# adammoss/nnest

Hardware: AMD Instinct MI355X
Metric: live-point evals/sec (flow-transform + loglike) + log-Z error, x_dim=50 (higher is better)
Workload: dtype f32

## Files before the change

### nnest_amd/csrc/nnest_train_grid.h

```cpp

enum { GRID_WG = 8, GRID_MAX_POLLS = 1 << 22 };

__device__ __forceinline__ void st_sc1_f32x4(float *p, f32x4 v) {
    asm volatile("global_store_dwordx4 %0, %1, off sc1\n\ts_nop 1" : : "v"(p), "v"(v) : "memory");
}
__device__ __forceinline__ float ld_sc1(const float *p) { return __hip_atomic_load(p, __ATOMIC_RELAXED, __HIP_MEMORY_SCOPE_AGENT); }
__device__ __forceinline__ f32x4 ld_sc1_x4_issue(const float *p) {
    f32x4 v;
    asm volatile("global_load_dwordx4 %0, %1, off sc1" : "=v"(v) : "v"(p) : "memory");
    return v;
}
__device__ __forceinline__ void st_sc1(float *p, float v) { __hip_atomic_store(p, v, __ATOMIC_RELAXED, __HIP_MEMORY_SCOPE_AGENT); }

__device__ __forceinline__ bool grid_barrier(unsigned int *ctr, int &phase, int G, int *err, int first_poll_sleep = 0) {
    asm volatile("s_waitcnt vmcnt(0)" ::: "memory");
    __syncthreads();
    phase += 1;
    __shared__ int ok;
    if (threadIdx.x == 0) {
        __hip_atomic_fetch_add(ctr, 1u, __ATOMIC_RELAXED, __HIP_MEMORY_SCOPE_AGENT);
        const unsigned int want = (unsigned int)G * (unsigned int)phase;
        int polls = 0, good = 1;
        if (first_poll_sleep >= 256) {
            for (int i = 256; i < first_poll_sleep; ++i) __builtin_amdgcn_s_sleep(4);
        } else if (first_poll_sleep > 8) __builtin_amdgcn_s_sleep(16);
        else if (first_poll_sleep > 0) __builtin_amdgcn_s_sleep(8);
        while (__hip_atomic_load(ctr, __ATOMIC_RELAXED, __HIP_MEMORY_SCOPE_AGENT) < want) {
            if (++polls > GRID_MAX_POLLS) { good = 0; *err = 1; break; }
            __builtin_amdgcn_s_sleep(1);
        }
        ok = good;
    }
    __syncthreads();
    return ok != 0;
}

template <int NT, int NH, int L>
__host__ __device__ inline void grid_job_targets(const FlowShape &s, int J, int lane, int r, int *wt, int *bt) {
    constexpr int J_W3 = NT * NH, J_W2 = L * NH * NH, NJOBS = J_W3 + J_W2 + NH * NT;
    const int D = s.D, H = s.H;
    const int bn = J / NJOBS, b = bn >> 1;
    int q = J % NJOBS;
    const int pc = (b + 1) & 1, pt = b & 1;
    const int pb0 = H * D, phid = H * D + H, pWo = H * D + H + L * (H * H + H), pbo = pWo + D * H;
    const int pbase = bn * s.net_params;
    const int gq = lane >> 4, j = lane & 15;
    *wt = -1; *bt = -1;
    if (q < J_W3) {
        const int tau = q / NH, ht = q % NH, d = 2 * (16 * tau + 4 * gq + r) + pt;
        if (d < D) {
            *wt = pbase + pWo + d * H + 16 * ht + j;
            if (ht == 0 && j == 0) *bt = pbase + pbo + d;
        }
        return;
    }
    q -= J_W3;
    if (q < J_W2) {
        const int l = q / (NH * NH) + 1, hto = (q / NH) % NH, hti = q % NH;
        *wt = pbase + phid + (l - 1) * (H * H + H) + (16 * hto + 4 * gq + r) * H + 16 * hti + j;
        if (hti == 0 && j == 0) *bt = pbase + phid + (l - 1) * (H * H + H) + H * H + 16 * hto + 4 * gq + r;
        return;
    }
    q -= J_W2;
    const int ht = q / NT, tau = q % NT, d = 2 * (16 * tau + j) + pc;
    if (d < D) *wt = pbase + (16 * ht + 4 * gq + r) * D + d;
    if (tau == 0 && j == 0) *bt = pbase + pb0 + 16 * ht + 4 * gq + r;
}

template <int NT, int NH, int L>
__global__ void grid_gpos_kernel(int *__restrict__ gpos, FlowShape s) {
    constexpr int NJOBS = NT * NH + L * NH * NH + NH * NT;
    const int NJ = s.B * 2 * NJOBS;
    for (int i = blockIdx.x * blockDim.x + threadIdx.x; i < NJ * 256; i += gridDim.x * blockDim.x) {
        const int J = i >> 8, lane = (i >> 2) & 63, r = i & 3;
        int wt, bt;
        grid_job_targets<NT, NH, L>(s, J, lane, r, &wt, &bt);
        if (wt >= 0) gpos[wt] = i;
        if (bt >= 0) gpos[bt] = NJ * 256 + i;
    }
}

template <int NT, int NH, int L>
__host__ __device__ inline void grid_job_image_offsets(const FlowShape &s, int J, int *off_f, int *off_b, int *off_bias) {
    constexpr int J_W3 = NT * NH, J_W2 = L * NH * NH, NJOBS = J_W3 + J_W2 + NH * NT;
    const int bn = J / NJOBS, base = bn * s.net_floats;
    int q = J % NJOBS;
    if (q < J_W3) {
        const int tau = q / NH, ht = q % NH;
        *off_b = base + frag_off_L1() + (ht * NT + tau) * 256;
        *off_f = base + frag_off_L3(NT, NH, L) + (tau * NH + ht) * 256;
        *off_bias = ht == 0 ? base + frag_off_b3(NT, NH, L) + 16 * tau : -1;
        return;
    }
    q -= J_W3;
    if (q < J_W2) {
        const int l = q / (NH * NH), hto = (q / NH) % NH, hti = q % NH;
        *off_b = base + frag_off_L2(NT, NH) + ((l * NH + hti) * NH + hto) * 256;
        *off_f = base + frag_off_L2(NT, NH) + ((l * NH + hto) * NH + hti) * 256;
        *off_bias = hti == 0 ? base + frag_off_b2(NT, NH, L) + l * 16 * NH + 16 * hto : -1;
        return;
    }
    q -= J_W2;
    const int ht = q / NT, tau = q % NT;
    *off_b = base + frag_off_L3(NT, NH, L) + (tau * NH + ht) * 256;
    *off_f = base + frag_off_L1() + (ht * NT + tau) * 256;
    *off_bias = tau == 0 ? base + frag_off_b1(NT, NH, L) + 16 * ht : -1;
}
__global__ void grid_dead_kernel(const int *__restrict__ gpos, int np, int *__restrict__ dead, int *__restrict__ count) {
    for (int p = blockIdx.x * blockDim.x + threadIdx.x; p < np; p += gridDim.x * blockDim.x)
        if (gpos[p] < 0) dead[atomicAdd(count, 1)] = p;
}

template <bool WITH_BIAS>
__device__ __forceinline__ f32x4 contract_rows_grid(const float *stg, int rows_pad, int ct_g, int ct_a, int lane, f32x4 &bias) {
    const f32x4 zero4 = {0.f, 0.f, 0.f, 0.f};
    f32x4 a0 = zero4, a1 = zero4, a2 = zero4, a3 = zero4;
    float bs = 0.f;
    const float *G = stg + (size_t)ct_g * TRAIN_MAX_ROWS * 16 + (lane >> 4) * 16 + (lane & 15);
    const float *A = stg + (size_t)ct_a * TRAIN_MAX_ROWS * 16 + (lane >> 4) * 16 + (lane & 15);
    constexpr int NIT = TRAIN_MAX_ROWS / 16;
    float gv[NIT][4], ev[NIT][4];
#pragma unroll
    for (int it = 0; it < NIT; ++it) {
        const int r = it * 16 < rows_pad ? it * 16 : 0;
#pragma unroll
        for (int k = 0; k < 4; ++k) {
            gv[it][k] = ld_sc1(G + (r + 4 * k) * 16);
            ev[it][k] = ld_sc1(A + (r + 4 * k) * 16);
        }
    }
#pragma unroll
    for (int it = 0; it < NIT; ++it) {
        if (it * 16 < rows_pad) {
            a0 = mfma4(gv[it][0], ev[it][0], a0);
            a1 = mfma4(gv[it][1], ev[it][1], a1);
            a2 = mfma4(gv[it][2], ev[it][2], a2);
            a3 = mfma4(gv[it][3], ev[it][3], a3);
            if (WITH_BIAS) bs += (gv[it][0] + gv[it][1]) + (gv[it][2] + gv[it][3]);
        }
    }
    if (WITH_BIAS) {
        bs += __shfl_xor(bs, 16);
        bs += __shfl_xor(bs, 32);
        const int q4 = (lane >> 4) * 4;
        bias = (f32x4){__shfl(bs, q4 + 0), __shfl(bs, q4 + 1), __shfl(bs, q4 + 2), __shfl(bs, q4 + 3)};
    }
    return (a0 + a1) + (a2 + a3);
}

__device__ __forceinline__ void stage_tile_grid(float *stg, int ct, int row, int lane, f32x4 v) {
    st_sc1_f32x4(stg + ((size_t)ct * TRAIN_MAX_ROWS + row) * 16 + (lane >> 4) * 4, v);
}

template <int NT, int NH, int L, int ACT>
__device__ __forceinline__ void mlp_bwd_grid(const float *__restrict__ bn, int lane, float *stg, int row, const f32x4 (&g_out)[NT],
                                             const f32x4 (&acts)[L + 1][NH], f32x4 (&g_m)[NT]) {
    typedef StageMap<NT, NH, L> SM;
    const float *B3 = bn + frag_off_L1() + 4 * lane;
    const float *B2 = bn + frag_off_L2(NT, NH) + 4 * lane;
    const float *B1 = bn + frag_off_L3(NT, NH, L) + 4 * lane;
    f32x4 gh[NH];
#pragma unroll
    for (int tau = 0; tau < NT; ++tau) stage_tile_grid(stg, SM::gout(tau), row, lane, g_out[tau]);
#pragma unroll
    for (int ht = 0; ht < NH; ++ht) {
        f32x4 acc = {0.f, 0.f, 0.f, 0.f};
#pragma unroll
        for (int tau = 0; tau < NT; ++tau) {
            const f32x4 f = frag_quad(B3, (ht * NT + tau));
            acc = mfma4(f.x, g_out[tau].x, acc);
            acc = mfma4(f.y, g_out[tau].y, acc);
            acc = mfma4(f.z, g_out[tau].z, acc);
            acc = mfma4(f.w, g_out[tau].w, acc);
        }
        gh[ht] = acc;
    }
#pragma unroll
    for (int l = L; l >= 1; --l) {
        f32x4 gpre[NH];
#pragma unroll
        for (int ht = 0; ht < NH; ++ht) {
            gpre[ht] = act_grad<ACT>(gh[ht], acts[l][ht]);
            stage_tile_grid(stg, SM::gpre(l, ht), row, lane, gpre[ht]);
            stage_tile_grid(stg, SM::act(l, ht), row, lane, acts[l][ht]);
        }
#pragma unroll
        for (int hti = 0; hti < NH; ++hti) {
            f32x4 acc = {0.f, 0.f, 0.f, 0.f};
#pragma unroll
            for (int hto = 0; hto < NH; ++hto) {
                const f32x4 f = frag_quad(B2, (((l - 1) * NH + hti) * NH + hto));
                acc = mfma4(f.x, gpre[hto].x, acc);
                acc = mfma4(f.y, gpre[hto].y, acc);
                acc = mfma4(f.z, gpre[hto].z, acc);
                acc = mfma4(f.w, gpre[hto].w, acc);
            }
            gh[hti] = acc;
        }
    }
    f32x4 gpre0[NH];
#pragma unroll
    for (int ht = 0; ht < NH; ++ht) {
        gpre0[ht] = act_grad<ACT>(gh[ht], acts[0][ht]);
        stage_tile_grid(stg, SM::gpre(0, ht), row, lane, gpre0[ht]);
        stage_tile_grid(stg, SM::act(0, ht), row, lane, acts[0][ht]);
    }
#pragma unroll
    for (int tau = 0; tau < NT; ++tau) {
        f32x4 acc = {0.f, 0.f, 0.f, 0.f};
#pragma unroll
        for (int ht = 0; ht < NH; ++ht) {
            const f32x4 f = frag_quad(B1, (tau * NH + ht));
            acc = mfma4(f.x, gpre0[ht].x, acc);
            acc = mfma4(f.y, gpre0[ht].y, acc);
            acc = mfma4(f.z, gpre0[ht].z, acc);
            acc = mfma4(f.w, gpre0[ht].w, acc);
        }
        g_m[tau] = acc;
    }
}

template <int NT, int NH, int L>
__device__ __forceinline__ void block_backward_grid(const TrainArgs &a, int b, int lane, int row, bool row_ok, const f32x4 (&cond)[NT],
                                                    f32x4 (&ytrans)[NT], f32x4 (&gcond)[NT], f32x4 (&gtrans)[NT], float gld,
                                                    const float *imgf, const float *imgb, const f32x4 *__restrict__ stash) {
    typedef StageMap<NT, NH, L> SM;
    const int pt = b & 1;
    const float *wf = imgf + (size_t)b * 2 * a.s.net_floats;
    const float *wb = imgb + (size_t)b * 2 * a.s.net_floats;
    float *stg_s = a.gstage + (size_t)(b * 2 + 0) * SM::count * TRAIN_MAX_ROWS * 16;
    float *stg_t = a.gstage + (size_t)(b * 2 + 1) * SM::count * TRAIN_MAX_ROWS * 16;
    f32x4 as[L + 1][NH], at[L + 1][NH], ls[NT], t[NT], g_ls[NT], g_t[NT], gm_s[NT], gm_t[NT];
    const int g = lane >> 4;
#pragma unroll
    for (int l = 0; l <= L; ++l)
#pragma unroll
        for (int ht = 0; ht < NH; ++ht) {
            as[l][ht] = stash[((0 * (L + 1) + l) * NH + ht) * 64 + lane];
            at[l][ht] = stash[((1 * (L + 1) + l) * NH + ht) * 64 + lane];
        }
    mlp_out_layer<NT, NH, L>(wf, lane, as[L], ls);
    mlp_out_layer<NT, NH, L>(wf + a.s.net_floats, lane, at[L], t);
#pragma unroll
    for (int tau = 0; tau < NT; ++tau) {
        float lsv[4] = {ls[tau].x, ls[tau].y, ls[tau].z, ls[tau].w};
        float tv[4] = {t[tau].x, t[tau].y, t[tau].z, t[tau].w};
        float yv[4] = {ytrans[tau].x, ytrans[tau].y, ytrans[tau].z, ytrans[tau].w};
        float gv[4] = {gtrans[tau].x, gtrans[tau].y, gtrans[tau].z, gtrans[tau].w};
        float o_gls[4], o_gt[4], o_x[4], o_gx[4];
#pragma unroll
        for (int r = 0; r < 4; ++r) {
            const int d = 2 * (16 * tau + 4 * g + r) + pt;
            const bool valid = row_ok && d < a.s.D;
            float ymt = yv[r] - tv[r];
            o_gls[r] = valid ? gv[r] * ymt + gld : 0.f;
            o_gt[r] = valid ? gv[r] : 0.f;
            o_x[r] = ymt * __expf(-lsv[r]);
            o_gx[r] = gv[r] * __expf(lsv[r]);
        }
        g_ls[tau] = (f32x4){o_gls[0], o_gls[1], o_gls[2], o_gls[3]};
        g_t[tau] = (f32x4){o_gt[0], o_gt[1], o_gt[2], o_gt[3]};
        ytrans[tau] = (f32x4){o_x[0], o_x[1], o_x[2], o_x[3]};
        gtrans[tau] = (f32x4){o_gx[0], o_gx[1], o_gx[2], o_gx[3]};
    }
    mlp_bwd_grid<NT, NH, L, 0>(wb, lane, stg_s, row, g_ls, as, gm_s);
#pragma unroll
    for (int tau = 0; tau < NT; ++tau) {
        f32x4 mv = cond[tau];
        if (!row_ok) mv = (f32x4){0.f, 0.f, 0.f, 0.f};
        stage_tile_grid(stg_s, SM::m(tau), row, lane, mv);
        stage_tile_grid(stg_t, SM::m(tau), row, lane, mv);
    }
    mlp_bwd_grid<NT, NH, L, 1>(wb + a.s.net_floats, lane, stg_t, row, g_t, at, gm_t);
#pragma unroll
    for (int tau = 0; tau < NT; ++tau) gcond[tau] = gcond[tau] + gm_s[tau] + gm_t[tau];
}

__device__ __forceinline__ void lds_barrier_t() { asm volatile("s_waitcnt lgkmcnt(0)\n\ts_barrier" ::: "memory"); }

template <int NT>
__device__ __forceinline__ void team_swap(f32x4 *xch, int role, int lane, const f32x4 (&mine)[NT], f32x4 (&other)[NT]) {
#pragma unroll
    for (int tau = 0; tau < NT; ++tau) xch[(role * NT + tau) * 64 + lane] = mine[tau];
// ... 571 lines not shown
```

### nnest_amd/csrc/nnest_train_rows.h

```cpp

enum { ROWS_PER_WG = 4, ROWS_B = 3 };

template <int U> struct RowsKeep {
    float h1, h2;
    float ls[(U + 1) / 2], tt[(U + 1) / 2];
};

__device__ __forceinline__ int rows_img_off(int b, int f, int lane) { return b * SOLO4_NF * 64 + ((f >> 2) * 64 + lane) * 4 + (f & 3); }

template <int U>
__device__ inline void rows_param_dest(int D, int b, int n, int o, int &df, int &db, bool &scaled) {
    const int cc = (b + 1) & 1, ct = b & 1;
    const int pb0 = 16 * D, pW1 = pb0 + 16, pb1 = pW1 + 256, pWo = pb1 + 16, pbo = pWo + 16 * D;
    df = db = -1;
    scaled = false;
    auto lane_of = [&](int pos, int src) { const int dl = (pos - src) & 15; return 32 * n + 16 * (dl >> 3) + pos; };
    auto rot_of = [&](int pos, int src) { return ((pos - src) & 15) & 7; };
    if (o < pb0) {
        const int j = o / D, d = o % D;
        if ((d & 1) != cc) return;
        const int s = d >> 1, q = s / U, u = s % U;
        df = rows_img_off(b, 8 * u + rot_of(j, q), lane_of(j, q));
        db = rows_img_off(b, 40 + 8 * u + rot_of(q, j), lane_of(q, j));
        scaled = n == 0;
// ... 100 lines not shown

static __device__ __forceinline__ float rows_act_grad(float g, float a, unsigned sel) {
    const float th = g * (1.f - a * a), rl = a > 0.f ? g : 0.f;
    unsigned out;
    asm("v_bfi_b32 %0, %1, %2, %3" : "=v"(out) : "v"(sel), "v"(__float_as_uint(rl)), "v"(__float_as_uint(th)));
    return __uint_as_float(out);
}

static __device__ __forceinline__ void rows_stage(float *stg_net, int ct, int row, int col, float v, bool stager) {
    if (stager) st_sc1(stg_net + ((size_t)ct * TRAIN_MAX_ROWS + row) * 16 + col, v);
}
template <int U>
static __device__ __forceinline__ void rows_stage_slots(float *stg_net, int ct0, int row, int pos, const float (&v)[U], bool stager) {
    if constexpr (U == 4) {
        const int s = 4 * pos;
        if (stager) st_sc1_f32x4(stg_net + ((size_t)(ct0 + (s >> 4)) * TRAIN_MAX_ROWS + row) * 16 + (s & 15), (f32x4){v[0], v[1], v[2], v[3]});
    } else {
#pragma unroll
        for (int u = 0; u < U; ++u) {
            const int s = U * pos + u;
            rows_stage(stg_net, ct0 + (s >> 4), row, s & 15, v[u], stager);
        }
    }
}

template <int U>
static __device__ __forceinline__ void rows_block_backward(const Solo4Lds &wb_, unsigned sel, bool h1, bool translate_half, int pos, int D, int ct,
                                                           bool row_ok, float gld, const float (&cond)[U], float (&ytrans)[U], float (&gcond)[U],
                                                           float (&gtrans)[U], const RowsKeep<U> &kp, float *stg_net, int row, bool stager) {
    typedef StageMap<U, 1, 1> SM;
    float go[U];
#pragma unroll
    for (int k = 0; k < U / 2; ++k) {
        const int u = 2 * k + (h1 ? 1 : 0);
        const bool valid = row_ok && 2 * U * pos + 2 * u + ct < D;
        const float yv = h1 ? ytrans[2 * k + 1] : ytrans[2 * k], gv = h1 ? gtrans[2 * k + 1] : gtrans[2 * k];
        const float ymt = yv - kp.tt[k];
        const float g_ls = valid ? gv * ymt + gld : 0.f, g_t = valid ? gv : 0.f;
        float x0 = ymt * __expf(-kp.ls[k]), gx0 = gv * __expf(kp.ls[k]), gs0 = translate_half ? g_t : g_ls;
        float x1 = x0, gx1 = gx0, gs1 = gs0;
        solo_swap16(x0, x1);
        solo_swap16(gx0, gx1);
        solo_swap16(gs0, gs1);
        ytrans[2 * k] = x0; ytrans[2 * k + 1] = x1;
        gtrans[2 * k] = gx0; gtrans[2 * k + 1] = gx1;
        go[2 * k] = gs0; go[2 * k + 1] = gs1;
    }
    if constexpr (U & 1) {
        const bool valid = row_ok && 2 * U * pos + 2 * (U - 1) + ct < D;
        const float gv = gtrans[U - 1], ymt = ytrans[U - 1] - kp.tt[U / 2];
        const float g_ls = valid ? gv * ymt + gld : 0.f, g_t = valid ? gv : 0.f;
        ytrans[U - 1] = ymt * __expf(-kp.ls[U / 2]);
        gtrans[U - 1] = gv * __expf(kp.ls[U / 2]);
        go[U - 1] = translate_half ? g_t : g_ls;
    }
    rows_stage_slots<U>(stg_net, SM::gout(0), row, pos, go, stager);
    float wa[8], wb[8], a0, a1;
    if constexpr (U >= 2) {
        wb_.load8(wa, 0); wb_.load8(wb, 8);
        solo_chain_2in(a0, a1, 0.f, solo_rot8_h1(go[0]), solo_rot8_h1(go[U >= 2 ? 1 : 0]), wa, wb);
    }
    if constexpr (U == 4) {
        wb_.load8(wa, 16); wb_.load8(wb, 24);
        solo_chain_2in_acc(a0, a1, solo_rot8_h1(go[U == 4 ? 2 : 0]), solo_rot8_h1(go[U == 4 ? 3 : 0]), wa, wb);
    }
    if constexpr (U == 1) {
        wb_.load8(wa, 0);
        solo_chain_1(a0, a1, 0.f, solo_rot8_h1(go[0]), wa);
    }
    if constexpr (U == 3) {
        wb_.load8(wa, 16);
        solo_chain_1_acc(a0, a1, solo_rot8_h1(go[U - 1]), wa);
    }
    float w2[8], w3a[8], w3b[8];
    wb_.load8(w2, 32);
    const float g_a2 = rows_act_grad(solo_join_rot(a0 + a1), kp.h2, sel);
    rows_stage(stg_net, SM::gpre(1, 0), row, pos, g_a2, stager);
    rows_stage(stg_net, SM::act(1, 0), row, pos, kp.h2, stager);
    if constexpr (U >= 2) { wb_.load8(w3a, 40); wb_.load8(w3b, 48); }
    solo_chain_1(a0, a1, 0.f, g_a2, w2);
    const float g_a1 = rows_act_grad(solo_join_rot(a0 + a1), kp.h1, sel);
    rows_stage(stg_net, SM::gpre(0, 0), row, pos, g_a1, stager);
    rows_stage(stg_net, SM::act(0, 0), row, pos, kp.h1, stager);
    {
        float cm[U];
#pragma unroll
        for (int u = 0; u < U; ++u) cm[u] = row_ok ? cond[u] : 0.f;
        rows_stage_slots<U>(stg_net, SM::m(0), row, pos, cm, stager);
    }
#pragma unroll
    for (int k = 0; k < U / 2; ++k) {
        float o0, o1;
        if (k > 0) { wb_.load8(w3a, 40 + 16 * k); wb_.load8(w3b, 48 + 16 * k); }
        solo_chain_2out(o0, o1, 0.f, 0.f, g_a1, w3a, w3b);
        solo_swap16(o0, o1);
        float fs, ft;
        solo_nets(o0 + o1, fs, ft);
        float t0 = fs + ft, t1 = t0;
        solo_swap16(t0, t1);
        gcond[2 * k] += t0;
        gcond[2 * k + 1] += t1;
    }
    if constexpr (U & 1) {
        float o0, o1;
        wb_.load8(wa, 40 + 8 * (U - 1));
        solo_chain_1(o0, o1, 0.f, g_a1, wa);
        float fs, ft;
        solo_nets(solo_join(o0 + o1), fs, ft);
        gcond[U - 1] += fs + ft;
    }
}

template <int U>
__device__ __forceinline__ void rows_prepare(const TrainArgs &a, int epoch, int mb, int wg, float *buf) {
    const int idx = (int)threadIdx.x - 64 * ROWS_PER_WG;
    if (idx < 0 || idx >= ROWS_PER_WG * 8 * U) return;
    const int r = idx / (8 * U), q = idx % (8 * U), D = a.s.D;
    const int M = min(a.batch, a.n_train - mb * a.batch);
    const int row = wg * ROWS_PER_WG + r;
    const bool row_ok = row < M;
    long src = 0;
    if (row_ok) src = a.perm[(size_t)epoch * a.n_train + mb * a.batch + row];
    const int d0 = 4 * q;
    float v[4];
#pragma unroll
    for (int j = 0; j < 4; ++j) v[j] = (row_ok && d0 + j < D) ? a.xtrain[(size_t)src * D + d0 + j] : 0.f;
    if (a.jitter != 0.f && row_ok) {
        const long p = (long)mb * a.batch + row;
        float n[4];
        if (a.noise) {
#pragma unroll
            for (int j = 0; j < 4; ++j) n[j] = d0 + j < D ? a.noise[((size_t)epoch * a.n_train + p) * D + d0 + j] : 0.f;
        } else {
            const f32x4 nn = noise_normal4(a.seed, (uint64_t)p, (uint32_t)(a.epoch_offset + epoch), (uint32_t)q, NOISE_STREAM_JITTER);
            n[0] = nn.x; n[1] = nn.y; n[2] = nn.z; n[3] = nn.w;
        }
#pragma unroll
        for (int j = 0; j < 4; ++j)
            if (d0 + j < D) v[j] += n[j] * a.jitter;
    }
    *reinterpret_cast<f32x4 *>(buf + r * 32 * U + d0) = (f32x4){v[0], v[1], v[2], v[3]};
}

template <int U>
__global__ void __launch_bounds__(TRAIN_THREADS) train_kernel_rows(TrainArgs a) {
    typedef StageMap<U, 1, 1> SM;
    constexpr int B = ROWS_B, IMG = ROWS_B * SOLO4_NF * 64;
    extern __shared__ __attribute__((aligned(16))) float smem[];
    float *imgf = smem;
    float *imgb = smem + IMG;
    __shared__ __attribute__((aligned(16))) float xpre[2][ROWS_PER_WG * 32 * U];
    __shared__ int ctl[4];
    __shared__ float ctlf[2];
    const int lane = threadIdx.x & 63, wave = threadIdx.x >> 6;
    const int pos = lane & 15;
    const bool h1 = (lane & 16) != 0, translate_half = lane >= 32, stager = (lane & 16) == 0;
    const int sl_r = (int)a.gld_in & 255, sl_b = ((int)a.gld_in >> 8) & 255;
    const unsigned sel = translate_half ? 0xffffffffu : 0u;
    const int wg = blockIdx.x, G = gridDim.x;
    const int D = a.s.D;
    constexpr int NJOBS = 2 * U + 1;
    const int NJ = B * 2 * NJOBS;
    int phase = 0;

    for (int i = threadIdx.x; i < 2 * IMG; i += blockDim.x) smem[i] = 0.f;
    __syncthreads();
    for (int p = threadIdx.x; p < a.s.nets_params(); p += blockDim.x) {
        const int bn = p / a.s.net_params, o = p - bn * a.s.net_params;
        int df, db; bool sc;
        rows_param_dest<U>(D, bn >> 1, bn & 1, o, df, db, sc);
        const float v = a.w[p];
        if (df >= 0) imgf[df] = sc ? SOLO_TANH_PRESCALE * v : v;
        if (db >= 0) imgb[db] = v;
    }
    constexpr int IMGF = ROWS_B * 2 * (2 * U * 256 + 256 + 16 + 16 + 16 * U);
    constexpr int RU = (IMGF / 4 + TRAIN_THREADS - 1) / TRAIN_THREADS;
    typedef int i32x4 __attribute__((ext_vector_type(4)));
    const i32x4 *gmap = reinterpret_cast<const i32x4 *>(a.gown);
    static_assert(2 * IMG < 0xffff && IMG < (1 << 14), "refresh map packing");

    const int Jmine = wave * G + wg;
    const bool owner = Jmine < NJ;
    int off_f = 0, off_b = 0, off_bias = -1;
    if (owner) grid_job_image_offsets<U, 1, 1>(a.s, Jmine, &off_f, &off_b, &off_bias);
    OwnState os;
#pragma unroll
    for (int r = 0; r < 4; ++r) {
        os.wt[r] = os.bt[r] = -1;
        os.tw[r] = os.tm[r] = os.tv[r] = os.bw[r] = os.bm[r] = os.bv[r] = 0.f;
    }
    if (owner) {
#pragma unroll
        for (int r = 0; r < 4; ++r) {
            grid_job_targets<U, 1, 1>(a.s, Jmine, lane, r, &os.wt[r], &os.bt[r]);
            if (os.wt[r] >= 0) { os.tw[r] = a.w[os.wt[r]]; os.tm[r] = a.m[os.wt[r]]; os.tv[r] = a.v[os.wt[r]]; }
            if (os.bt[r] >= 0) { os.bw[r] = a.w[os.bt[r]]; os.bm[r] = a.m[os.bt[r]]; os.bv[r] = a.v[os.bt[r]]; }
        }
    }
    const int n_waves = G * TRAIN_WAVES, ndead = *a.gndead;
    const int ndead_pad = (ndead + 63) & ~63;
    const int dead_per = ((ndead + n_waves - 1) / n_waves + 63) & ~63;
    const int dead0 = min(ndead, Jmine * dead_per), dead1 = min(ndead, dead0 + dead_per);
    float *dw = a.gdst, *dm = a.gdst + ndead_pad, *dv = a.gdst + 2 * ndead_pad;
    for (int k = dead0 + lane; k < dead1; k += 64) {
        const int pidx = a.gdead[k];
        dw[k] = a.w[pidx]; dm[k] = a.m[pidx]; dv[k] = a.v[pidx];
    }
    const bool resume = (a.flags & NNEST_TRAIN_RESUME) != 0;
    if (threadIdx.x == 0) {
        ctl[0] = 0;
        ctl[1] = resume ? a.result->counter : 0;
        ctl[2] = resume ? a.result->best_epoch : 0;
        ctlf[0] = resume ? a.result->best_validation_loss : INFINITY;
    }
    if (!resume) {
        if (owner) {
#pragma unroll
            for (int r = 0; r < 4; ++r) {
                if (os.wt[r] >= 0) st_sc1(a.best_w + os.wt[r], os.tw[r]);
                if (os.bt[r] >= 0) st_sc1(a.best_w + os.bt[r], os.bw[r]);
            }
        }
        for (int k = dead0 + lane; k < dead1; k += 64) st_sc1(a.best_w + a.gdead[k], dw[k]);
    }
    const int n_mb = (a.n_train + a.batch - 1) / a.batch;
    if (a.max_epochs > 0) rows_prepare<U>(a, 0, 0, wg, xpre[0]);
    __syncthreads();

    float *pub = a.gimgf;
    float *part_base = a.gtile;
    auto sum_rows = [&](const float *words) {
        float v = (lane < ROWS_PER_WG * G ? ld_sc1(words + lane) : 0.f) + (lane + 64 < ROWS_PER_WG * G ? ld_sc1(words + lane + 64) : 0.f);
#pragma unroll
        for (int o = 1; o < 64; o <<= 1) v += __shfl_xor(v, o);
        return v;
    };
    int adam_t = a.adam_step ? *a.adam_step : 0;
    unsigned long long ph[8] = {0, 0, 0, 0, 0, 0, 0, 0}, q0 = 0, q1 = 0, q2 = 0, q3 = 0, q4 = 0, q5 = 0, q6 = 0;
    (void)ph; (void)q0; (void)q1; (void)q2; (void)q3; (void)q4; (void)q5; (void)q6;
    int epochs_run = 0, mbcount = 0;
    float last_train_loss = 0.f;
    bool alive = true;
    unsigned long long dbg_arr = 0, dbg_st = 0;
    (void)dbg_arr; (void)dbg_st;
    const int row = wg * ROWS_PER_WG + wave;
    float *stg_net0 = a.gstage + (size_t)(translate_half ? 1 : 0) * SM::count * TRAIN_MAX_ROWS * 16;

    auto forward = [&](float (&xs)[2][U], RowsKeep<U> (&kp)[B]) {
        float ld = rows_block_forward<U>(Solo4Lds{imgf, lane}, sel, h1, xs[1], xs[0], kp[0]);
        ld += rows_block_forward<U>(Solo4Lds{imgf + SOLO4_NF * 64, lane}, sel, h1, xs[0], xs[1], kp[1]);
        ld += rows_block_forward<U>(Solo4Lds{imgf + 2 * SOLO4_NF * 64, lane}, sel, h1, xs[1], xs[0], kp[2]);
        return ld;
    };
    auto log_prob = [&](const float (&xs)[2][U], float ld_lane) {
        float ss = 0.f;
#pragma unroll
        for (int c = 0; c < 2; ++c)
#pragma unroll
            for (int u = 0; u < U; ++u) ss += base_E(xs[c][u], a.s.base_beta);
        return -solo_row_sum(ss) + a.s.base_const * (float)D + solo_logdet_total(ld_lane);
    };

    for (int epoch = 0; epoch < a.max_epochs && alive; ++epoch) {
        float epoch_loss = 0.f;
        for (int mb = 0; mb < n_mb && alive; ++mb, ++mbcount) {
            const int M = min(a.batch, a.n_train - mb * a.batch);
            const int rows_pad = ((M + 15) >> 4) * 16;
            const bool row_ok = wave < ROWS_PER_WG && row < M;
            float *part = part_base + (mbcount & 1) * TRAIN_MAX_ROWS;
            AdamStep ad;
            {
                adam_t += 1;
                const double bc1 = 1.0 - pow(0.9, (double)adam_t), bc2 = 1.0 - pow(0.999, (double)adam_t);
                ad.step_size = (float)((double)a.lr / bc1);
                ad.inv_bc2s = (float)(1.0 / sqrt(bc2));
            }
            TSTAMP(q0);
#ifdef NNEST_STAMP
            const unsigned long long rt_start = __builtin_amdgcn_s_memrealtime();
#endif
            {
                int e2 = epoch, m2 = mb + 1;
                if (m2 == n_mb) { m2 = 0; e2 = epoch + 1; }
                if (e2 < a.max_epochs) rows_prepare<U>(a, e2, m2, wg, xpre[(mbcount + 1) & 1]);
            }
            if (wave < ROWS_PER_WG) {
                float lp = 0.f;
                if (row < rows_pad) {
                    float xs[2][U], gs[2][U];
                    const float *xr = xpre[mbcount & 1] + wave * 32 * U + 2 * U * pos;
#pragma unroll
                    for (int u = 0; u < U; ++u) { xs[0][u] = xr[2 * u]; xs[1][u] = xr[2 * u + 1]; }
                    RowsKeep<U> kp[B];
                    const float ld_lane = forward(xs, kp);
                    lp = row_ok ? log_prob(xs, ld_lane) : 0.f;
                    TSTAMP(q1);
                    const float invM = 1.0f / (float)M, gld = -invM;
#pragma unroll
                    for (int c = 0; c < 2; ++c)
#pragma unroll
                        for (int u = 0; u < U; ++u) gs[c][u] = row_ok ? base_dE(xs[c][u], a.s.base_beta) * invM : 0.f;
                    constexpr size_t RS = (size_t)2 * SM::count * TRAIN_MAX_ROWS * 16;
                    rows_block_backward<U>(Solo4Lds{imgb + 2 * SOLO4_NF * 64, lane}, sel, h1, translate_half, pos, D, 0, row_ok, gld, xs[1], xs[0], gs[1], gs[0], kp[2], stg_net0 + 2 * RS, row, stager);
                    rows_block_backward<U>(Solo4Lds{imgb + SOLO4_NF * 64, lane}, sel, h1, translate_half, pos, D, 1, row_ok, gld, xs[0], xs[1], gs[0], gs[1], kp[1], stg_net0 + RS, row, stager);
                    rows_block_backward<U>(Solo4Lds{imgb, lane}, sel, h1, translate_half, pos, D, 0, row_ok, gld, xs[1], xs[0], gs[1], gs[0], kp[0], stg_net0, row, stager);
                }
                if (lane == 0) st_sc1(part + row, lp);
            }
            TSTAMP(q2);
#ifdef NNEST_STAMP
            if (mbcount == 20) { dbg_arr = __builtin_amdgcn_s_memrealtime(); dbg_st = rt_start; }
#endif
#ifdef NNEST_STAMP
            {
                unsigned long long s0 = 0, s1 = 0;
                TSTAMP(s0);
                asm volatile("s_waitcnt vmcnt(0)" ::: "memory");
                __syncthreads();
                TSTAMP(s1);
                phase += 1;
                __shared__ int okd;
                if (threadIdx.x == 0) {
                    __hip_atomic_fetch_add(a.gsync, 1u, __ATOMIC_RELAXED, __HIP_MEMORY_SCOPE_AGENT);
                    const unsigned int want = (unsigned int)G * (unsigned int)phase;
                    int polls = 0;
                    __builtin_amdgcn_s_sleep(16);
                    while (__hip_atomic_load(a.gsync, __ATOMIC_RELAXED, __HIP_MEMORY_SCOPE_AGENT) < want) { ++polls; __builtin_amdgcn_s_sleep(1); }
                    okd = 1;
                    TACC(ph[6], s1, s0);
                    ph[7] += polls;
                }
                __syncthreads();
                alive = okd != 0;
            }
#else
            alive = grid_barrier(a.gsync, phase, G, a.gerr, 256 + sl_b);
#endif
            if (!alive) break;
            TSTAMP(q3);
            if (owner) {
                const int J = Jmine;
                const int bn = J / NJOBS;
                int q = J % NJOBS;
                const float *stg = a.gstage + (size_t)bn * SM::count * TRAIN_MAX_ROWS * 16;
                f32x4 bt = {0.f, 0.f, 0.f, 0.f}, t;
                constexpr int J_W3 = U, J_W2 = 1;
                if (q < J_W3) {
                    t = contract_rows_grid<true>(stg, rows_pad, SM::gout(q), SM::act(1, 0), lane, bt);
                } else if (q - J_W3 < J_W2) {
                    t = contract_rows_grid<true>(stg, rows_pad, SM::gpre(1, 0), SM::act(0, 0), lane, bt);
                } else {
                    q -= J_W3 + J_W2;
                    t = q == 0 ? contract_rows_grid<true>(stg, rows_pad, SM::gpre(0, 0), SM::m(q), lane, bt)
                               : contract_rows_grid<false>(stg, rows_pad, SM::gpre(0, 0), SM::m(q), lane, bt);
                }
                const float gt[4] = {t.x, t.y, t.z, t.w}, gb[4] = {bt.x, bt.y, bt.z, bt.w};
#pragma unroll
                for (int r = 0; r < 4; ++r) {
                    if (os.wt[r] >= 0) adam_reg(a, ad, os.tw[r], gt[r], os.tm[r], os.tv[r]);
                    if (os.bt[r] >= 0) adam_reg(a, ad, os.bw[r], gb[r], os.bm[r], os.bv[r]);
                }
                const float tg = __int_as_float(mbcount + 1);
                st_sc1_f32x4(pub + 2 * (off_b + lane * 4), (f32x4){os.tw[0], tg, os.tw[1], tg});
                st_sc1_f32x4(pub + 2 * (off_b + lane * 4) + 4, (f32x4){os.tw[2], tg, os.tw[3], tg});
                if (off_bias >= 0 && (lane & 15) == 0) {
                    st_sc1_f32x4(pub + 2 * (off_bias + (lane >> 4) * 4), (f32x4){os.bw[0], tg, os.bw[1], tg});
                    st_sc1_f32x4(pub + 2 * (off_bias + (lane >> 4) * 4) + 4, (f32x4){os.bw[2], tg, os.bw[3], tg});
                }
            }
            for (int k = dead0 + lane; k < dead1; k += 64) {
                float w_ = dw[k], m_ = dm[k], v_ = dv[k];
                adam_reg(a, ad, w_, 0.f, m_, v_);
                dw[k] = w_; dm[k] = m_; dv[k] = v_;
            }
            TSTAMP(q4);
            __syncthreads();
            TSTAMP(q5);
            float lsum = 0.f;
            if (wave == 0) lsum = sum_rows(part);
            {
                constexpr int CH = RU > 4 ? 4 : RU;
                const int want = mbcount + 1;
                for (int i = 0; i < sl_r; ++i) __builtin_amdgcn_s_sleep(4);
#pragma unroll
                for (int c0 = 0; c0 < RU; c0 += CH) {
                    f32x4 va[CH], vc[CH];
                    i32x4 mp[CH];
#pragma unroll
                    for (int u = 0; u < CH; ++u) mp[u] = gmap[min((int)threadIdx.x + (c0 + u) * TRAIN_THREADS, IMGF / 4 - 1)];
                    bool fresh = false;
                    for (int polls = 0; !fresh; ++polls) {
                        if (polls > GRID_MAX_POLLS / 64) { *a.gerr = 1; break; }
#pragma unroll
                        for (int u = 0; u < CH; ++u) {
                            const int i = min((int)threadIdx.x + (c0 + u) * TRAIN_THREADS, IMGF / 4 - 1);
                            va[u] = ld_sc1_x4_issue(pub + 8 * (size_t)i);
                            vc[u] = ld_sc1_x4_issue(pub + 8 * (size_t)i + 4);
                        }
#pragma unroll
                        for (int u = 0; u < CH; ++u) asm volatile("s_waitcnt vmcnt(0)" : "+v"(va[u]), "+v"(vc[u]) : : "memory");
                        fresh = true;
#pragma unroll
                        for (int u = 0; u < CH; ++u)
                            fresh = fresh && __float_as_int(va[u].y) == want && __float_as_int(va[u].w) == want && __float_as_int(vc[u].y) == want &&
                                    __float_as_int(vc[u].w) == want;
                    }
#pragma unroll
                    for (int u = 0; u < CH; ++u) {
                        if (c0 + u < RU && (int)threadIdx.x + (c0 + u) * TRAIN_THREADS < IMGF / 4) {
                            const float e4[4] = {va[u].x, va[u].z, vc[u].x, vc[u].z};
                            const int m4[4] = {mp[u].x, mp[u].y, mp[u].z, mp[u].w};
#pragma unroll
                            for (int e = 0; e < 4; ++e) {
                                const int f = m4[e] & 0xffff, k = (m4[e] >> 16) & 0xffff;
                                if (f != 0xffff) smem[f & 0x3fff] = (f >> 14) ? SOLO_TANH_PRESCALE * e4[e] : e4[e];
                                if (k != 0xffff) smem[k] = e4[e];
                            }
                        }
                    }
                }
            }
            epoch_loss += -lsum / (float)M;
            alive = __syncthreads_and(*a.gerr == 0 ? 1 : 0) != 0;
            if (!alive) break;
            TSTAMP(q6);
            if (wave == 0 && q1 > q0) { TACC(ph[0], q1, q0); TACC(ph[1], q2, q1); }
            TACC(ph[2], q3, q2); TACC(ph[3], q4, q3); TACC(ph[4], q5, q4); TACC(ph[5], q6, q5);
        }
        if (!alive) break;
        {
            float vsum = 0.f;
            if (wave < ROWS_PER_WG) {
                for (int r = row; r < a.n_valid; r += ROWS_PER_WG * G) {
                    float xs[2][U];
#pragma unroll
                    for (int u = 0; u < U; ++u)
#pragma unroll
                        for (int c = 0; c < 2; ++c) {
                            const int d = 2 * U * pos + 2 * u + c;
                            xs[c][u] = d < D ? a.xvalid[(size_t)r * D + d] : 0.f;
                        }
                    RowsKeep<U> kp[B];
                    const float ld_lane = forward(xs, kp);
                    vsum += log_prob(xs, ld_lane);
                }
                if (lane == 0) st_sc1(part_base + (2 + (epoch & 1)) * TRAIN_MAX_ROWS + row, vsum);
            }
            alive = grid_barrier(a.gsync, phase, G, a.gerr);
            if (!alive) break;
            const float vtot = sum_rows(part_base + (2 + (epoch & 1)) * TRAIN_MAX_ROWS);
            const float valid_loss = (-vtot / (float)a.n_valid) / (float)a.n_valid;
            const float train_loss = epoch_loss / (float)a.n_train;
            last_train_loss = train_loss;
            epochs_run = epoch + 1;
#ifndef NNEST_STAMP
            if (a.losses && wg == 0 && threadIdx.x == 0) {
                a.losses[2 * epoch] = train_loss;
                a.losses[2 * epoch + 1] = valid_loss;
            }
#endif
            const bool improved = valid_loss < ctlf[0];
            __syncthreads();
            if (improved) {
                if (owner) {
#pragma unroll
                    for (int r = 0; r < 4; ++r) {
                        if (os.wt[r] >= 0) st_sc1(a.best_w + os.wt[r], os.tw[r]);
                        if (os.bt[r] >= 0) st_sc1(a.best_w + os.bt[r], os.bw[r]);
                    }
                }
                for (int k = dead0 + lane; k < dead1; k += 64) st_sc1(a.best_w + a.gdead[k], dw[k]);
                if (threadIdx.x == 0) { ctlf[0] = valid_loss; ctl[2] = a.epoch_offset + epoch + 1; ctl[1] = 0; }
            }
            __syncthreads();
            if (threadIdx.x == 0) {
                ctl[1] += 1;
                if (ctl[1] > a.patience) ctl[0] = 1;
            }
            __syncthreads();
            if (ctl[0]) break;
        }
    }
#ifdef NNEST_STAMP
    if (threadIdx.x == 0 && a.losses && wg < 28) {
        a.losses[20 + wg] = (float)(dbg_arr & 0xffffff);
        a.losses[50 + wg] = (float)(dbg_st & 0xffffff);
    }
#endif
    __syncthreads();
    const bool stopped = ctl[0] != 0;
    const bool restore = stopped || (a.flags & NNEST_TRAIN_FINALIZE);
    if (owner) {
#pragma unroll
        for (int r = 0; r < 4; ++r) {
            if (os.wt[r] >= 0) {
                st_sc1(a.w + os.wt[r], restore ? ld_sc1(a.best_w + os.wt[r]) : os.tw[r]);
                st_sc1(a.m + os.wt[r], os.tm[r]); st_sc1(a.v + os.wt[r], os.tv[r]);
            }
            if (os.bt[r] >= 0) {
                st_sc1(a.w + os.bt[r], restore ? ld_sc1(a.best_w + os.bt[r]) : os.bw[r]);
                st_sc1(a.m + os.bt[r], os.bm[r]); st_sc1(a.v + os.bt[r], os.bv[r]);
            }
        }
    }
    for (int k = dead0 + lane; k < dead1; k += 64) {
        const int pidx = a.gdead[k];
        st_sc1(a.w + pidx, restore ? ld_sc1(a.best_w + pidx) : dw[k]);
        st_sc1(a.m + pidx, dm[k]); st_sc1(a.v + pidx, dv[k]);
    }
    if (wg != 0) return;
#ifdef NNEST_STAMP
    if (threadIdx.x == 0 && a.losses)
        for (int i = 0; i < 8; ++i) a.losses[i] = (float)ph[i];
#endif
    if (threadIdx.x == 0) {
        if (a.adam_step) *a.adam_step = adam_t;
        a.result->epochs_run = a.epoch_offset + epochs_run;
        a.result->best_epoch = ctl[2];
        a.result->best_validation_loss = ctlf[0];
        a.result->last_train_loss = last_train_loss;
        a.result->counter = ctl[1];
        a.result->stopped = *a.gerr ? 2 : (stopped ? 1 : 0);
    }
}

static bool rows_eligible(const TrainArgs &a) {
    static const bool off = [] { const char *e = getenv("NNEST_TRAIN_FORM"); return e && !strcmp(e, "grid"); }();
    return !off && a.s.H == 16 && a.s.NH == 1 && a.s.L == 1 && a.s.B == ROWS_B && a.s.NT >= 1 && a.s.NT <= 4 && a.batch >= 1 &&
           a.batch <= TRAIN_MAX_ROWS;
}

template <int U>
static hipError_t launch_train_rows_t(TrainArgs a, float *gridws, hipStream_t st) {
    typedef GridSizes<U, 1, 1> GS;
    a.gstage = gridws;
    a.gtile = a.gstage + GS::stage(a.s);
    a.gpos = reinterpret_cast<int *>(a.gtile + GS::tiles(a.s));
    a.gpart = reinterpret_cast<float *>(a.gpos + a.s.num_params());
    a.gsync = reinterpret_cast<unsigned int *>(a.gpart + 64);
    a.gerr = reinterpret_cast<int *>(a.gsync + 8);
    a.gndead = reinterpret_cast<int *>(a.gsync + 12);
    a.gdead = reinterpret_cast<int *>(a.gpart + 64 + 16);
    a.gown = reinterpret_cast<float *>(a.gdead + a.s.num_params());
    a.gown += (64 - ((size_t)(a.gown - gridws) & 63)) & 63;
    a.gdst = a.gown + (size_t)GRID_WG * TRAIN_WAVES * 64 * 32;
    a.gimgf = a.gdst + (size_t)3 * ((a.s.num_params() + 63) & ~63) + 64;
    a.gimgf += (64 - ((size_t)(a.gimgf - gridws) & 63)) & 63;
    a.gimgb = a.gimgf + ((a.s.image_floats + 63) & ~63);
    hipError_t e = hipMemsetAsync(a.gstage, 0, GS::stage(a.s) * sizeof(float), st);
    if (e != hipSuccess) return e;
    e = hipMemsetAsync(a.gpos, 0xFF, (size_t)a.s.num_params() * sizeof(int), st);
    if (e != hipSuccess) return e;
    e = hipMemsetAsync(a.gimgf, 0, (size_t)2 * ((a.s.image_floats + 63) & ~63) * sizeof(float), st);
    if (e != hipSuccess) return e;
    e = hipMemsetAsync(a.gpart, 0, (64 + 16) * sizeof(float), st);
    if (e != hipSuccess) return e;
    hipLaunchKernelGGL((grid_gpos_kernel<U, 1, 1>), dim3(32), dim3(256), 0, st, a.gpos, a.s);
    hipLaunchKernelGGL(grid_dead_kernel, dim3(32), dim3(256), 0, st, a.gpos, a.s.num_params(), a.gdead, a.gndead);
    hipLaunchKernelGGL((rows_maps_kernel<U>), dim3(32), dim3(256), 0, st, reinterpret_cast<int *>(a.gown), a.s);
    {
        const int r = 4, b = 4;
        a.gld_in = (float)(r + 256 * b);
    }
    const int NJ = ROWS_B * 2 * (2 * U + 1);
    const int G = max((a.batch + ROWS_PER_WG - 1) / ROWS_PER_WG, (NJ + TRAIN_WAVES - 1) / TRAIN_WAVES);
    const size_t lds = (size_t)2 * ROWS_B * SOLO4_NF * 64 * sizeof(float);
    e = hipFuncSetAttribute(reinterpret_cast<const void *>(train_kernel_rows<U>), hipFuncAttributeMaxDynamicSharedMemorySize, (int)lds);
    if (e != hipSuccess) return e;
    hipLaunchKernelGGL((train_kernel_rows<U>), dim3(G), dim3(TRAIN_THREADS), lds, st, a);
    e = hipGetLastError();
    if (e != hipSuccess) return e;
    return launch_repack(a.w, a.img_fwd, a.s, st);
}

static hipError_t dispatch_train_rows(const TrainArgs &a, float *gridws, hipStream_t st) {
    switch (a.s.NT) {
        case 1: return launch_train_rows_t<1>(a, gridws, st);
        case 2: return launch_train_rows_t<2>(a, gridws, st);
        case 3: return launch_train_rows_t<3>(a, gridws, st);
        case 4: return launch_train_rows_t<4>(a, gridws, st);
    }
    return hipErrorInvalidConfiguration;
}
```

Measured before the change: 915.9 million.

## Overlap dead-param Adam and bias-correction scalars with grid barrier wait

Inlines the grid barrier into the rows training kernel, so that after arriving at the counter the waves do the dead-parameter Adam updates and precompute the next step's bias-correction scalars (double-buffered in shared memory) while thread 0 polls. Dead-parameter work is remapped onto the waves least loaded with owner jobs, and the loss-partial loads are issued before the image polling loop, so their latency is hidden. The error flag is also read early rather than after the final sync. These steps hide latency, at the cost of more instrumentation and a different error-check ordering. An environment variable can now override the hold/sleep parameters.

```diff
diff --git a/nnest_amd/csrc/nnest_train_grid.h b/nnest_amd/csrc/nnest_train_grid.h
--- a/nnest_amd/csrc/nnest_train_grid.h
+++ b/nnest_amd/csrc/nnest_train_grid.h
@@ -112,7 +112,8 @@
 }
 
 template <bool WITH_BIAS>
-__device__ __forceinline__ f32x4 contract_rows_grid(const float *stg, int rows_pad, int ct_g, int ct_a, int lane, f32x4 &bias) {
+__device__ __forceinline__ f32x4 contract_rows_grid(const float *stg, int rows_pad, int ct_g, int ct_a, int lane, f32x4 &bias,
+                                                    unsigned long long *t_requested = nullptr, unsigned long long *t_landed = nullptr) {
     const f32x4 zero4 = {0.f, 0.f, 0.f, 0.f};
     f32x4 a0 = zero4, a1 = zero4, a2 = zero4, a3 = zero4;
     float bs = 0.f;
@@ -129,6 +130,13 @@
             ev[it][k] = ld_sc1(A + (r + 4 * k) * 16);
         }
     }
+#ifdef NNEST_STAMP
+    if (t_requested) {
+        TSTAMP(*t_requested);
+        asm volatile("s_waitcnt vmcnt(0)" ::: "memory");
+        TSTAMP(*t_landed);
+    }
+#endif
 #pragma unroll
     for (int it = 0; it < NIT; ++it) {
         if (it * 16 < rows_pad) {
diff --git a/nnest_amd/csrc/nnest_train_rows.h b/nnest_amd/csrc/nnest_train_rows.h
--- a/nnest_amd/csrc/nnest_train_rows.h
+++ b/nnest_amd/csrc/nnest_train_rows.h
@@ -276,6 +276,8 @@
     __shared__ __attribute__((aligned(16))) float xpre[2][ROWS_PER_WG * 32 * U];
     __shared__ int ctl[4];
     __shared__ float ctlf[2];
+    __shared__ float adsc[2][2];
+    __shared__ int bar_ok;
     const int lane = threadIdx.x & 63, wave = threadIdx.x >> 6;
     const int pos = lane & 15;
     const bool h1 = (lane & 16) != 0, translate_half = lane >= 32, stager = (lane & 16) == 0;
@@ -324,7 +326,8 @@
     const int n_waves = G * TRAIN_WAVES, ndead = *a.gndead;
     const int ndead_pad = (ndead + 63) & ~63;
     const int dead_per = ((ndead + n_waves - 1) / n_waves + 63) & ~63;
-    const int dead0 = min(ndead, Jmine * dead_per), dead1 = min(ndead, dead0 + dead_per);
+    const int Jdead = (TRAIN_WAVES - 1 - wave) * G + wg;
+    const int dead0 = min(ndead, Jdead * dead_per), dead1 = min(ndead, dead0 + dead_per);
     float *dw = a.gdst, *dm = a.gdst + ndead_pad, *dv = a.gdst + 2 * ndead_pad;
     for (int k = dead0 + lane; k < dead1; k += 64) {
         const int pidx = a.gdead[k];
@@ -349,6 +352,14 @@
     }
     const int n_mb = (a.n_train + a.batch - 1) / a.batch;
     if (a.max_epochs > 0) rows_prepare<U>(a, 0, 0, wg, xpre[0]);
+    int adam_t = a.adam_step ? *a.adam_step : 0;
+    auto adam_scalars = [&](int t, float *slot) {
+        const double bc1 = 1.0 - pow(0.9, (double)t), bc2 = 1.0 - pow(0.999, (double)t);
+        slot[0] = (float)((double)a.lr / bc1);
+        slot[1] = (float)(1.0 / sqrt(bc2));
+    };
+    const bool scalar_thread = threadIdx.x == 64 * (TRAIN_WAVES - 1);
+    if (scalar_thread) adam_scalars(adam_t + 1, adsc[0]);
     __syncthreads();
 
     float *pub = a.gimgf;
@@ -359,9 +370,9 @@
         for (int o = 1; o < 64; o <<= 1) v += __shfl_xor(v, o);
         return v;
     };
-    int adam_t = a.adam_step ? *a.adam_step : 0;
-    unsigned long long ph[8] = {0, 0, 0, 0, 0, 0, 0, 0}, q0 = 0, q1 = 0, q2 = 0, q3 = 0, q4 = 0, q5 = 0, q6 = 0;
-    (void)ph; (void)q0; (void)q1; (void)q2; (void)q3; (void)q4; (void)q5; (void)q6;
+    unsigned long long ph[16] = {0, 0, 0, 0, 0, 0, 0, 0, 0, 0, 0, 0, 0, 0, 0, 0}, q0 = 0, q1 = 0, q2 = 0, q3 = 0, q4 = 0, q5 = 0, q6 = 0;
+    unsigned long long j1 = 0, j2 = 0, r1 = 0, r2 = 0, r3 = 0;
+    (void)ph; (void)q0; (void)q1; (void)q2; (void)q3; (void)q4; (void)q5; (void)q6; (void)j1; (void)j2; (void)r1; (void)r2; (void)r3;
     int epochs_run = 0, mbcount = 0;
     float last_train_loss = 0.f;
     bool alive = true;
@@ -392,15 +403,10 @@
             const int rows_pad = ((M + 15) >> 4) * 16;
             const bool row_ok = wave < ROWS_PER_WG && row < M;
             float *part = part_base + (mbcount & 1) * TRAIN_MAX_ROWS;
-            AdamStep ad;
-            {
-                adam_t += 1;
-                const double bc1 = 1.0 - pow(0.9, (double)adam_t), bc2 = 1.0 - pow(0.999, (double)adam_t);
-                ad.step_size = (float)((double)a.lr / bc1);
-                ad.inv_bc2s = (float)(1.0 / sqrt(bc2));
-            }
+            adam_t += 1;
             TSTAMP(q0);
 #ifdef NNEST_STAMP
+            if (q6 != 0) TACC(ph[8], q0, q6);
             const unsigned long long rt_start = __builtin_amdgcn_s_memrealtime();
 #endif
             {
@@ -435,31 +441,42 @@
 #ifdef NNEST_STAMP
             if (mbcount == 20) { dbg_arr = __builtin_amdgcn_s_memrealtime(); dbg_st = rt_start; }
 #endif
-#ifdef NNEST_STAMP
+            AdamStep ad;
             {
                 unsigned long long s0 = 0, s1 = 0;
+                (void)s0; (void)s1;
                 TSTAMP(s0);
                 asm volatile("s_waitcnt vmcnt(0)" ::: "memory");
                 __syncthreads();
                 TSTAMP(s1);
                 phase += 1;
-                __shared__ int okd;
+                if (threadIdx.x == 0) __hip_atomic_fetch_add(a.gsync, 1u, __ATOMIC_RELAXED, __HIP_MEMORY_SCOPE_AGENT);
+                asm volatile("" ::: "memory");
+                ad.step_size = adsc[mbcount & 1][0];
+                ad.inv_bc2s = adsc[mbcount & 1][1];
+                for (int k = dead0 + lane; k < dead1; k += 64) {
+                    float w_ = dw[k], m_ = dm[k], v_ = dv[k];
+                    adam_reg(a, ad, w_, 0.f, m_, v_);
+                    dw[k] = w_; dm[k] = m_; dv[k] = v_;
+                }
+                if (scalar_thread) adam_scalars(adam_t + 1, adsc[(mbcount + 1) & 1]);
                 if (threadIdx.x == 0) {
-                    __hip_atomic_fetch_add(a.gsync, 1u, __ATOMIC_RELAXED, __HIP_MEMORY_SCOPE_AGENT);
                     const unsigned int want = (unsigned int)G * (unsigned int)phase;
-                    int polls = 0;
-                    __builtin_amdgcn_s_sleep(16);
-                    while (__hip_atomic_load(a.gsync, __ATOMIC_RELAXED, __HIP_MEMORY_SCOPE_AGENT) < want) { ++polls; __builtin_amdgcn_s_sleep(1); }
-                    okd = 1;
+                    int polls = 0, good = 1;
+                    for (int i = 0; i < sl_b; ++i) __builtin_amdgcn_s_sleep(4);
+                    while (__hip_atomic_load(a.gsync, __ATOMIC_RELAXED, __HIP_MEMORY_SCOPE_AGENT) < want) {
+                        if (++polls > GRID_MAX_POLLS) { good = 0; *a.gerr = 1; break; }
+                        __builtin_amdgcn_s_sleep(1);
+                    }
+                    bar_ok = good;
                     TACC(ph[6], s1, s0);
+#ifdef NNEST_STAMP
                     ph[7] += polls;
+#endif
                 }
                 __syncthreads();
-                alive = okd != 0;
-            }
-#else
-            alive = grid_barrier(a.gsync, phase, G, a.gerr, 256 + sl_b);
-#endif
+                alive = bar_ok != 0;
+            }
             if (!alive) break;
             TSTAMP(q3);
             if (owner) {
@@ -470,13 +487,13 @@
                 f32x4 bt = {0.f, 0.f, 0.f, 0.f}, t;
                 constexpr int J_W3 = U, J_W2 = 1;
                 if (q < J_W3) {
-                    t = contract_rows_grid<true>(stg, rows_pad, SM::gout(q), SM::act(1, 0), lane, bt);
+                    t = contract_rows_grid<true>(stg, rows_pad, SM::gout(q), SM::act(1, 0), lane, bt, &j1, &j2);
                 } else if (q - J_W3 < J_W2) {
-                    t = contract_rows_grid<true>(stg, rows_pad, SM::gpre(1, 0), SM::act(0, 0), lane, bt);
+                    t = contract_rows_grid<true>(stg, rows_pad, SM::gpre(1, 0), SM::act(0, 0), lane, bt, &j1, &j2);
                 } else {
                     q -= J_W3 + J_W2;
-                    t = q == 0 ? contract_rows_grid<true>(stg, rows_pad, SM::gpre(0, 0), SM::m(q), lane, bt)
-                               : contract_rows_grid<false>(stg, rows_pad, SM::gpre(0, 0), SM::m(q), lane, bt);
+                    t = q == 0 ? contract_rows_grid<true>(stg, rows_pad, SM::gpre(0, 0), SM::m(q), lane, bt, &j1, &j2)
+                               : contract_rows_grid<false>(stg, rows_pad, SM::gpre(0, 0), SM::m(q), lane, bt, &j1, &j2);
                 }
                 const float gt[4] = {t.x, t.y, t.z, t.w}, gb[4] = {bt.x, bt.y, bt.z, bt.w};
 #pragma unroll
@@ -492,16 +509,16 @@
                     st_sc1_f32x4(pub + 2 * (off_bias + (lane >> 4) * 4) + 4, (f32x4){os.bw[2], tg, os.bw[3], tg});
                 }
             }
-            for (int k = dead0 + lane; k < dead1; k += 64) {
-                float w_ = dw[k], m_ = dm[k], v_ = dv[k];
-                adam_reg(a, ad, w_, 0.f, m_, v_);
-                dw[k] = w_; dm[k] = m_; dv[k] = v_;
-            }
             TSTAMP(q4);
             __syncthreads();
             TSTAMP(q5);
-            float lsum = 0.f;
-            if (wave == 0) lsum = sum_rows(part);
+            float lw0 = 0.f, lw1 = 0.f;
+            if (wave == 0) {
+                if (lane < ROWS_PER_WG * G) lw0 = ld_sc1(part + lane);
+                if (lane + 64 < ROWS_PER_WG * G) lw1 = ld_sc1(part + lane + 64);
+            }
+            const int err_seen = __hip_atomic_load(a.gerr, __ATOMIC_RELAXED, __HIP_MEMORY_SCOPE_AGENT);
+            bool ran_out = false;
             {
                 constexpr int CH = RU > 4 ? 4 : RU;
                 const int want = mbcount + 1;
@@ -514,13 +531,16 @@
                     for (int u = 0; u < CH; ++u) mp[u] = gmap[min((int)threadIdx.x + (c0 + u) * TRAIN_THREADS, IMGF / 4 - 1)];
                     bool fresh = false;
                     for (int polls = 0; !fresh; ++polls) {
-                        if (polls > GRID_MAX_POLLS / 64) { *a.gerr = 1; break; }
+                        if (polls > GRID_MAX_POLLS / 64) { *a.gerr = 1; ran_out = true; break; }
 #pragma unroll
                         for (int u = 0; u < CH; ++u) {
                             const int i = min((int)threadIdx.x + (c0 + u) * TRAIN_THREADS, IMGF / 4 - 1);
                             va[u] = ld_sc1_x4_issue(pub + 8 * (size_t)i);
                             vc[u] = ld_sc1_x4_issue(pub + 8 * (size_t)i + 4);
                         }
+#ifdef NNEST_STAMP
+                        if (c0 == 0 && polls == 0) TSTAMP(r1);
+#endif
 #pragma unroll
                         for (int u = 0; u < CH; ++u) asm volatile("s_waitcnt vmcnt(0)" : "+v"(va[u]), "+v"(vc[u]) : : "memory");
                         fresh = true;
@@ -529,6 +549,7 @@
                             fresh = fresh && __float_as_int(va[u].y) == want && __float_as_int(va[u].w) == want && __float_as_int(vc[u].y) == want &&
                                     __float_as_int(vc[u].w) == want;
                     }
+                    if (c0 + CH >= RU) TSTAMP(r2);
 #pragma unroll
                     for (int u = 0; u < CH; ++u) {
                         if (c0 + u < RU && (int)threadIdx.x + (c0 + u) * TRAIN_THREADS < IMGF / 4) {
@@ -544,12 +565,21 @@
                     }
                 }
             }
+            TSTAMP(r3);
+            asm volatile("" : "+v"(lw0), "+v"(lw1));
+            float lsum = lw0 + lw1;
+            if (wave == 0) {
+#pragma unroll
+                for (int o = 1; o < 64; o <<= 1) lsum += __shfl_xor(lsum, o);
+            }
             epoch_loss += -lsum / (float)M;
-            alive = __syncthreads_and(*a.gerr == 0 ? 1 : 0) != 0;
+            alive = __syncthreads_and(err_seen == 0 && !ran_out ? 1 : 0) != 0;
             if (!alive) break;
             TSTAMP(q6);
             if (wave == 0 && q1 > q0) { TACC(ph[0], q1, q0); TACC(ph[1], q2, q1); }
             TACC(ph[2], q3, q2); TACC(ph[3], q4, q3); TACC(ph[4], q5, q4); TACC(ph[5], q6, q5);
+            TACC(ph[9], j1, q3); TACC(ph[10], j2, j1); TACC(ph[11], q4, j2);
+            TACC(ph[12], r1, q5); TACC(ph[13], r2, r1); TACC(ph[14], r3, r2); TACC(ph[15], q6, r3);
         }
         if (!alive) break;
         {
@@ -577,6 +607,9 @@
             const float train_loss = epoch_loss / (float)a.n_train;
             last_train_loss = train_loss;
             epochs_run = epoch + 1;
+#ifdef NNEST_STAMP
+            q6 = 0;
+#endif
 #ifndef NNEST_STAMP
             if (a.losses && wg == 0 && threadIdx.x == 0) {
                 a.losses[2 * epoch] = train_loss;
@@ -635,7 +668,7 @@
     if (wg != 0) return;
 #ifdef NNEST_STAMP
     if (threadIdx.x == 0 && a.losses)
-        for (int i = 0; i < 8; ++i) a.losses[i] = (float)ph[i];
+        for (int i = 0; i < 16; ++i) a.losses[i] = (float)ph[i];
 #endif
     if (threadIdx.x == 0) {
         if (a.adam_step) *a.adam_step = adam_t;
@@ -683,8 +716,15 @@
     hipLaunchKernelGGL(grid_dead_kernel, dim3(32), dim3(256), 0, st, a.gpos, a.s.num_params(), a.gdead, a.gndead);
     hipLaunchKernelGGL((rows_maps_kernel<U>), dim3(32), dim3(256), 0, st, reinterpret_cast<int *>(a.gown), a.s);
     {
-        const int r = 4, b = 4;
-        a.gld_in = (float)(r + 256 * b);
+        static const int hold = [] {
+            int r = 4, b = 4;
+            if (const char *e = getenv("NNEST_ROWS_HOLD")) {
+                r = atoi(e);
+                if (const char *c = strchr(e, ',')) b = atoi(c + 1);
+            }
+            return (r & 255) + 256 * (b & 255);
+        }();
+        a.gld_in = (float)hold;
     }
     const int NJ = ROWS_B * 2 * (2 * U + 1);
     const int G = max((a.batch + ROWS_PER_WG - 1) / ROWS_PER_WG, (NJ + TRAIN_WAVES - 1) / TRAIN_WAVES);
```

New measurement: 915.0 million. About the same (-0.1%).
